# tencent-ailab/V-Express

Measured on AMD Instinct MI355X. Metric: decoded frames/sec at 512x512, 25 DDIM steps, higher is better.
Workload: dtype bf16; 1 GPU; 512x512, 16 frames (1 window(s) of 16, overlap 4), 25 DDIM steps, CFG 3.5, random-init UNet3D + ReferenceNet banks + sd-vae-ft-mse decode; frames=16, windows=1, parallelism=window x CFG-half units over 1 GPU(s)

## Files before the change

### v-express_amd/csrc/vx_norm.hip

```cpp
#include "vx_common.h"
#include "vx_gemm_common.h"
#include "../../include/vexpress_hip.h"

namespace {

constexpr int GN_THREADS = 256;
constexpr int GN_MAX_SETS = 2;

constexpr int GN_UNROLL = 4;
constexpr int GN_SUBS = 8;

struct GnPlan {
  const bf16_t* base[GN_MAX_SETS];
  int pstride[GN_MAX_SETS];
  int chunk[GN_MAX_SETS];
  int pl, pl_count;
};

__device__ __forceinline__ GnPlan gn_plan(const bf16_t* x1, int c1, const bf16_t* x2, int c2, int hw, int frame) {
  GnPlan P;
  const int nchunks = (c1 + c2) >> 3;
  const int tid = threadIdx.x;
  const int tp = nchunks < GN_THREADS ? nchunks : GN_THREADS;
  P.pl_count = GN_THREADS / tp;
  const int cc = tid % tp;
  P.pl = tid / tp;
  const bool active = P.pl < P.pl_count;
#pragma unroll
  for (int u = 0; u < GN_MAX_SETS; ++u) {
    const int chunk = cc + u * GN_THREADS;
    P.chunk[u] = chunk;
    const int ch = chunk * 8;
    if (active && chunk < nchunks) {
      if (ch < c1) {
        P.base[u] = x1 + (size_t)frame * hw * c1 + ch;
        P.pstride[u] = c1;
      } else {
        P.base[u] = x2 + (size_t)frame * hw * c2 + (ch - c1);
        P.pstride[u] = c2;
      }
    } else {
      P.base[u] = nullptr;
      P.pstride[u] = 0;
    }
  }
  return P;
}

__global__ __launch_bounds__(GN_THREADS) void gn_stats_kernel(const bf16_t* __restrict__ x1, int c1,
                                                              const bf16_t* __restrict__ x2, int c2, int hw,
                                                              int groups, int slices, int slice_pix,
                                                              float* __restrict__ ws) {
  extern __shared__ __attribute__((aligned(16))) char smem[];
  const int C = c1 + c2;
  const int bid = VX_XCD_ROWS ? xcd_remap(blockIdx.x, gridDim.x) : (int)blockIdx.x;
  const int frame = bid / slices, slice = bid % slices;
  const int tid = threadIdx.x;
  const GnPlan P = gn_plan(x1, c1, x2, c2, hw, frame);
  const int p_begin = slice * slice_pix;
  const int p_end = min(hw, p_begin + slice_pix);

  float s[GN_MAX_SETS][8], q[GN_MAX_SETS][8];
#pragma unroll
  for (int u = 0; u < GN_MAX_SETS; ++u)
#pragma unroll
    for (int e = 0; e < 8; ++e) s[u][e] = q[u][e] = 0.f;

#pragma unroll
  for (int u = 0; u < GN_MAX_SETS; ++u) {
    if (P.base[u] == nullptr) continue;
    const bf16_t* src = P.base[u];
    const int ps = P.pstride[u];
    int px = p_begin + P.pl;
    for (; px + (GN_UNROLL - 1) * P.pl_count < p_end; px += GN_UNROLL * P.pl_count) {
      uint4 raw[GN_UNROLL];
#pragma unroll
      for (int k = 0; k < GN_UNROLL; ++k)
        raw[k] = *reinterpret_cast<const uint4*>(src + (size_t)(px + k * P.pl_count) * ps);
#pragma unroll
      for (int k = 0; k < GN_UNROLL; ++k) {
        float f[8];
        unpack_bf16x8(raw[k], f);
#pragma unroll
        for (int e = 0; e < 8; ++e) {
          s[u][e] += f[e];
          q[u][e] += f[e] * f[e];
        }
      }
    }
    for (; px < p_end; px += P.pl_count) {
      float f[8];
      unpack_bf16x8(*reinterpret_cast<const uint4*>(src + (size_t)px * ps), f);
#pragma unroll
      for (int e = 0; e < 8; ++e) {
        s[u][e] += f[e];
        q[u][e] += f[e] * f[e];
      }
    }
  }
  float* part = reinterpret_cast<float*>(smem);
#pragma unroll
  for (int u = 0; u < GN_MAX_SETS; ++u) {
    if (P.base[u] == nullptr) continue;
#pragma unroll
    for (int e = 0; e < 8; ++e) {
      part[((size_t)P.pl * C + P.chunk[u] * 8 + e) * 2 + 0] = s[u][e];
      part[((size_t)P.pl * C + P.chunk[u] * 8 + e) * 2 + 1] = q[u][e];
    }
  }
  __syncthreads();
  for (int ch = tid; ch < C; ch += GN_THREADS) {
    float a = 0.f, b = 0.f;
    for (int l = 0; l < P.pl_count; ++l) {
      a += part[((size_t)l * C + ch) * 2 + 0];
      b += part[((size_t)l * C + ch) * 2 + 1];
    }
    part[(size_t)ch * 2 + 0] = a;
    part[(size_t)ch * 2 + 1] = b;
  }
  __syncthreads();
  const int cg = C / groups;
  for (int g = tid; g < groups; g += GN_THREADS) {
    float a = 0.f, b = 0.f;
    for (int j = 0; j < cg; ++j) {
      a += part[(size_t)(g * cg + j) * 2 + 0];
      b += part[(size_t)(g * cg + j) * 2 + 1];
    }
    float* o = ws + (((size_t)frame * slices + slice) * groups + g) * 2;
    o[0] = a;
    o[1] = b;
  }
}

__device__ __forceinline__ void gn_group_stats(const float* __restrict__ ws, int frame, int slices, int groups, int cg,
                                               int hw, float eps, float* gstat, double* dpart) {
  const int tid = threadIdx.x;
  for (int idx = tid; idx < groups * GN_SUBS; idx += GN_THREADS) {
    const int g = idx % groups, sub = idx / groups;
    double a = 0.0, b = 0.0;
    for (int sl = sub; sl < slices; sl += GN_SUBS) {
      const float2 o = *reinterpret_cast<const float2*>(ws + (((size_t)frame * slices + sl) * groups + g) * 2);
      a += (double)o.x;
      b += (double)o.y;
    }
    dpart[(sub * groups + g) * 2 + 0] = a;
    dpart[(sub * groups + g) * 2 + 1] = b;
  }
  __syncthreads();
  for (int g = tid; g < groups; g += GN_THREADS) {
    double a = 0.0, b = 0.0;
    for (int sub = 0; sub < GN_SUBS; ++sub) {
      a += dpart[(sub * groups + g) * 2 + 0];
      b += dpart[(sub * groups + g) * 2 + 1];
    }
    double cnt = (double)cg * (double)hw;
    double mean = a / cnt;
    double var = b / cnt - mean * mean;
    if (var < 0.0) var = 0.0;
    gstat[g * 2 + 0] = (float)mean;
    gstat[g * 2 + 1] = (float)(1.0 / sqrt(var + (double)eps));
  }
  __syncthreads();
}

constexpr int GN_FOLD_ROWS = GN_THREADS / 8;
__global__ __launch_bounds__(GN_THREADS) void gn_fold_linear_kernel(const float* __restrict__ ws, int hw, int slices,
                                                                    int groups, float eps,
                                                                    const float* __restrict__ gamma, int C,
                                                                    const bf16_t* __restrict__ w,
                                                                    const float* __restrict__ bias_beta, int n,
                                                                    bf16_t* __restrict__ w_out,
                                                                    float* __restrict__ bias_out) {
  extern __shared__ __attribute__((aligned(16))) char smem[];
  const int frame = blockIdx.y, tid = threadIdx.x;
  float* scale = reinterpret_cast<float*>(smem);
  float* meanc = scale + C;
  float* gstat = meanc + C;
  double* dpart = reinterpret_cast<double*>(gstat + 2 * groups);
  const int cg = C / groups;
  gn_group_stats(ws, frame, slices, groups, cg, hw, eps, gstat, dpart);
  for (int ch = tid; ch < C; ch += GN_THREADS) {
    const int g = ch / cg;
    scale[ch] = gamma[ch] * gstat[g * 2 + 1];
    meanc[ch] = gstat[g * 2 + 0];
  }
  __syncthreads();
  const int row = blockIdx.x * GN_FOLD_ROWS + (tid >> 3), sub = tid & 7;
  float dot = 0.f;
  if (row < n) {
    const bf16_t* src = w + (size_t)row * C;
    bf16_t* dst = w_out + ((size_t)frame * n + row) * C;
    for (int ch = sub * 8; ch < C; ch += 64) {
      float f[8];
      unpack_bf16x8(*reinterpret_cast<const uint4*>(src + ch), f);
#pragma unroll
      for (int e = 0; e < 8; ++e) f[e] *= scale[ch + e];
      const uint4 pk = pack_bf16x8(f);
      *reinterpret_cast<uint4*>(dst + ch) = pk;
      unpack_bf16x8(pk, f);
#pragma unroll
      for (int e = 0; e < 8; ++e) dot = fmaf(f[e], meanc[ch + e], dot);
    }
  }
  dot = wave_xor_sum(dot, 1);
  dot = wave_xor_sum(dot, 2);
  dot = wave_xor_sum(dot, 4);
  if (row < n && sub == 0) bias_out[(size_t)frame * n + row] = bias_beta[row] - dot;
}

__global__ __launch_bounds__(GN_THREADS) void gn_apply_kernel(const bf16_t* __restrict__ x1, int c1,
                                                              const bf16_t* __restrict__ x2, int c2, int hw,
                                                              int groups, float eps, const float* __restrict__ gamma,
                                                              const float* __restrict__ beta, int silu,
                                                              bf16_t* __restrict__ out, int slices, int slice_pix,
                                                              const float* __restrict__ ws, int width, int w_shift,
                                                              int out_pad, int stat_slices) {
  extern __shared__ __attribute__((aligned(16))) char smem[];
  const int C = c1 + c2;
  const int bid = VX_XCD_ROWS ? xcd_remap(blockIdx.x, gridDim.x) : (int)blockIdx.x;
  const int frame = bid / slices, slice = bid % slices;
  const int tid = threadIdx.x;
  float* scale = reinterpret_cast<float*>(smem);
  float* shift = scale + C;
  float* gstat = shift + C;
  double* dpart = reinterpret_cast<double*>(gstat + 2 * groups);
  const int cg = C / groups;
  gn_group_stats(ws, frame, stat_slices, groups, cg, hw, eps, gstat, dpart);
  for (int ch = tid; ch < C; ch += GN_THREADS) {
    int g = ch / cg;
    float sc = gamma[ch] * gstat[g * 2 + 1];
    scale[ch] = sc;
    shift[ch] = beta[ch] - gstat[g * 2 + 0] * sc;
  }
  __syncthreads();
  const GnPlan P = gn_plan(x1, c1, x2, c2, hw, frame);
  const int p_begin = slice * slice_pix;
  const int p_end = min(hw, p_begin + slice_pix);
  const int wp = width + 2 * out_pad;
  const int hp = hw / width + 2 * out_pad;
  bf16_t* const oframe = out + (size_t)frame * hp * wp * C;
  auto opix = [&](int px) {
    if (out_pad == 0) return px;
    const int y = w_shift >= 0 ? px >> w_shift : px / width;
    return (y + out_pad) * wp + (px - y * width) + out_pad;
  };
#pragma unroll
  for (int u = 0; u < GN_MAX_SETS; ++u) {
    if (P.base[u] == nullptr) continue;
    const bf16_t* src = P.base[u];
    const int ps = P.pstride[u];
    const int ch = P.chunk[u] * 8;
    float sc[8], sh[8];
#pragma unroll
    for (int e = 0; e < 8; ++e) {
      sc[e] = scale[ch + e];
      sh[e] = shift[ch + e];
    }
    auto emit = [&](const uint4& raw, int px) {
      float f[8];
      unpack_bf16x8(raw, f);
#pragma unroll
      for (int e = 0; e < 8; ++e) f[e] = f[e] * sc[e] + sh[e];
      if (silu == 1) {
#pragma unroll
        for (int e = 0; e < 8; ++e) f[e] = silu_f(f[e]);
      } else if (silu == 2) {
#pragma unroll
        for (int e = 0; e < 8; ++e) f[e] = gelu_f(f[e]);
      }
      *reinterpret_cast<uint4*>(oframe + (size_t)opix(px) * C + ch) = pack_bf16x8(f);
    };
    int px = p_begin + P.pl;
    for (; px + (GN_UNROLL - 1) * P.pl_count < p_end; px += GN_UNROLL * P.pl_count) {
      uint4 raw[GN_UNROLL];
#pragma unroll
      for (int k = 0; k < GN_UNROLL; ++k)
        raw[k] = *reinterpret_cast<const uint4*>(src + (size_t)(px + k * P.pl_count) * ps);
#pragma unroll
      for (int k = 0; k < GN_UNROLL; ++k) emit(raw[k], px + k * P.pl_count);
    }
    for (; px < p_end; px += P.pl_count) emit(*reinterpret_cast<const uint4*>(src + (size_t)px * ps), px);
  }
}

constexpr int LN_R = 4;

template <int MAXC>
__global__ __launch_bounds__(256) void layernorm_kernel(const bf16_t* __restrict__ x, int ldx, int rows, int c,
                                                        float eps, const float* __restrict__ gamma,
                                                        const float* __restrict__ beta,
                                                        const float* __restrict__ add, int add_rows_per_entry,
                                                        int add_entries, bf16_t* __restrict__ out, int ldo) {
  const int lane = threadIdx.x & 63;
  const int wave = blockIdx.x * 4 + (threadIdx.x >> 6);
  const int nwaves = gridDim.x * 4;
  const int nchunks = c >> 3;
  const float inv_c = 1.0f / (float)c;
  bool live[MAXC];
  float g[MAXC][8], b[MAXC][8];
#pragma unroll
  for (int u = 0; u < MAXC; ++u) {
    const int chunk = lane + u * 64;
    live[u] = chunk < nchunks;
    const int cs = live[u] ? chunk : 0;
    const float4 g0 = *reinterpret_cast<const float4*>(gamma + cs * 8);
    const float4 g1 = *reinterpret_cast<const float4*>(gamma + cs * 8 + 4);
    const float4 b0 = *reinterpret_cast<const float4*>(beta + cs * 8);
    const float4 b1 = *reinterpret_cast<const float4*>(beta + cs * 8 + 4);
    g[u][0] = g0.x; g[u][1] = g0.y; g[u][2] = g0.z; g[u][3] = g0.w;
    g[u][4] = g1.x; g[u][5] = g1.y; g[u][6] = g1.z; g[u][7] = g1.w;
    b[u][0] = b0.x; b[u][1] = b0.y; b[u][2] = b0.z; b[u][3] = b0.w;
    b[u][4] = b1.x; b[u][5] = b1.y; b[u][6] = b1.z; b[u][7] = b1.w;
  }
  for (int row0 = wave * LN_R; row0 < rows; row0 += nwaves * LN_R) {
    uint4 raw[LN_R][MAXC];
#pragma unroll
    for (int r = 0; r < LN_R; ++r) {
      const int row = min(row0 + r, rows - 1);
#pragma unroll
      for (int u = 0; u < MAXC; ++u) {
        const int chunk = live[u] ? lane + u * 64 : 0;
        raw[r][u] = *reinterpret_cast<const uint4*>(x + (size_t)row * ldx + chunk * 8);
      }
    }
    float sum[LN_R];
#pragma unroll
    for (int r = 0; r < LN_R; ++r) {
      sum[r] = 0.f;
#pragma unroll
      for (int u = 0; u < MAXC; ++u) {
        float v[8];
        unpack_bf16x8(raw[r][u], v);
        float t = ((v[0] + v[1]) + (v[2] + v[3])) + ((v[4] + v[5]) + (v[6] + v[7]));
        sum[r] += live[u] ? t : 0.f;
      }
    }
#pragma unroll
    for (int m = 32; m >= 1; m >>= 1)
#pragma unroll
      for (int r = 0; r < LN_R; ++r) sum[r] = wave_xor_sum(sum[r], m);
    float sq[LN_R];
#pragma unroll
    for (int r = 0; r < LN_R; ++r) {
      const float mean = sum[r] * inv_c;
      sq[r] = 0.f;
#pragma unroll
      for (int u = 0; u < MAXC; ++u) {
        float v[8];
        unpack_bf16x8(raw[r][u], v);
        float t = 0.f;
#pragma unroll
        for (int e = 0; e < 8; ++e) {
          const float d = v[e] - mean;
          t += d * d;
        }
        sq[r] += live[u] ? t : 0.f;
      }
    }
#pragma unroll
    for (int m = 32; m >= 1; m >>= 1)
#pragma unroll
      for (int r = 0; r < LN_R; ++r) sq[r] = wave_xor_sum(sq[r], m);
#pragma unroll
    for (int r = 0; r < LN_R; ++r) {
      const int row = row0 + r;
      if (row >= rows) break;
      const float mean = sum[r] * inv_c;
      const float rstd = rsqrtf(sq[r] * inv_c + eps);
      const float* addrow = nullptr;
      if (add != nullptr) addrow = add + (size_t)((row / add_rows_per_entry) % add_entries) * c;
#pragma unroll
      for (int u = 0; u < MAXC; ++u) {
        if (!live[u]) continue;
        const int chunk = lane + u * 64;
        float v[8], o[8];
        unpack_bf16x8(raw[r][u], v);
#pragma unroll
        for (int e = 0; e < 8; ++e) o[e] = (v[e] - mean) * rstd * g[u][e] + b[u][e];
        if (addrow != nullptr) {
          const float4 a0 = *reinterpret_cast<const float4*>(addrow + chunk * 8);
          const float4 a1 = *reinterpret_cast<const float4*>(addrow + chunk * 8 + 4);
          o[0] += a0.x; o[1] += a0.y; o[2] += a0.z; o[3] += a0.w;
          o[4] += a1.x; o[5] += a1.y; o[6] += a1.z; o[7] += a1.w;
        }
        *reinterpret_cast<uint4*>(out + (size_t)row * ldo + chunk * 8) = pack_bf16x8(o);
      }
    }
  }
}

template <int MAXC>
__global__ __launch_bounds__(256) void row_stats_kernel(const bf16_t* __restrict__ x, int ldx, int rows, int c, float eps,
                                                        float2* __restrict__ stats) {
  const int lane = threadIdx.x & 63;
  const int wave = blockIdx.x * 4 + (threadIdx.x >> 6);
  const int nwaves = gridDim.x * 4;
  const int nchunks = c >> 3;
  const float inv_c = 1.0f / (float)c;
  for (int row0 = wave * LN_R; row0 < rows; row0 += nwaves * LN_R) {
    uint4 raw[LN_R][MAXC];
#pragma unroll
    for (int r = 0; r < LN_R; ++r) {
      const int row = min(row0 + r, rows - 1);
#pragma unroll
      for (int u = 0; u < MAXC; ++u) {
        const int chunk = lane + u * 64 < nchunks ? lane + u * 64 : 0;
        raw[r][u] = *reinterpret_cast<const uint4*>(x + (size_t)row * ldx + chunk * 8);
      }
    }
    float sum[LN_R];
#pragma unroll
    for (int r = 0; r < LN_R; ++r) {
      sum[r] = 0.f;
#pragma unroll
      for (int u = 0; u < MAXC; ++u) {
        float v[8];
        unpack_bf16x8(raw[r][u], v);
        const float t = ((v[0] + v[1]) + (v[2] + v[3])) + ((v[4] + v[5]) + (v[6] + v[7]));
        sum[r] += lane + u * 64 < nchunks ? t : 0.f;
      }
    }
#pragma unroll
    for (int m = 32; m >= 1; m >>= 1)
#pragma unroll
      for (int r = 0; r < LN_R; ++r) sum[r] = wave_xor_sum(sum[r], m);
    float sq[LN_R];
#pragma unroll
    for (int r = 0; r < LN_R; ++r) {
      const float mean = sum[r] * inv_c;
      sq[r] = 0.f;
#pragma unroll
      for (int u = 0; u < MAXC; ++u) {
        float v[8];
        unpack_bf16x8(raw[r][u], v);
        float t = 0.f;
#pragma unroll
        for (int e = 0; e < 8; ++e) {
          const float d = v[e] - mean;
          t += d * d;
        }
        sq[r] += lane + u * 64 < nchunks ? t : 0.f;
      }
    }
#pragma unroll
    for (int m = 32; m >= 1; m >>= 1)
#pragma unroll
      for (int r = 0; r < LN_R; ++r) sq[r] = wave_xor_sum(sq[r], m);
    if (lane < LN_R && row0 + lane < rows) {
      float mean = 0.f, var = 0.f;
#pragma unroll
      for (int r = 0; r < LN_R; ++r)
        if (lane == r) {
          mean = sum[r] * inv_c;
          var = sq[r] * inv_c;
        }
      stats[row0 + lane] = make_float2(mean, rsqrtf(var + eps));
    }
  }
}

template <int MAXC, bool NORM>
__global__ __launch_bounds__(256) void layernorm_fp8_kernel(const bf16_t* __restrict__ x, int ldx, int rows, int c,
                                                            float eps, const float* __restrict__ gamma,
                                                            const float* __restrict__ beta,
                                                            const float* __restrict__ add, int add_rows_per_entry,
                                                            int add_entries, uint8_t* __restrict__ out8, int ldo8,
                                                            float* __restrict__ scale) {
  const int lane = threadIdx.x & 63;
  const int wave = blockIdx.x * 4 + (threadIdx.x >> 6);
  const int nwaves = gridDim.x * 4;
  const int nchunks = c >> 3, ochunks = ldo8 >> 3;
  const float inv_c = 1.0f / (float)c;
  for (int row = wave; row < rows; row += nwaves) {
    float y[MAXC][8];
    float sum = 0.f;
#pragma unroll
    for (int u = 0; u < MAXC; ++u) {
      const int chunk = lane + u * 64;
      if (chunk < nchunks) {
        unpack_bf16x8(*reinterpret_cast<const uint4*>(x + (size_t)row * ldx + chunk * 8), y[u]);
      } else {
#pragma unroll
        for (int e = 0; e < 8; ++e) y[u][e] = 0.f;
      }
      sum += ((y[u][0] + y[u][1]) + (y[u][2] + y[u][3])) + ((y[u][4] + y[u][5]) + (y[u][6] + y[u][7]));
    }
    if (NORM) {
#pragma unroll
      for (int m = 32; m >= 1; m >>= 1) sum = wave_xor_sum(sum, m);
      const float mean = sum * inv_c;
      float sq = 0.f;
#pragma unroll
      for (int u = 0; u < MAXC; ++u) {
        if (lane + u * 64 < nchunks) {
#pragma unroll
          for (int e = 0; e < 8; ++e) {
            const float d = y[u][e] - mean;
            sq += d * d;
          }
        }
      }
#pragma unroll
      for (int m = 32; m >= 1; m >>= 1) sq = wave_xor_sum(sq, m);
      const float rstd = rsqrtf(sq * inv_c + eps);
      const float* addrow = add != nullptr ? add + (size_t)((row / add_rows_per_entry) % add_entries) * c : nullptr;
#pragma unroll
      for (int u = 0; u < MAXC; ++u) {
        const int chunk = lane + u * 64;
        if (chunk < nchunks) {
#pragma unroll
          for (int e = 0; e < 8; ++e) {
            float o = (y[u][e] - mean) * rstd * gamma[chunk * 8 + e] + beta[chunk * 8 + e];
            if (addrow != nullptr) o += addrow[chunk * 8 + e];
            y[u][e] = o;
          }
        }
      }
    }
    float amax = 0.f;
#pragma unroll
    for (int u = 0; u < MAXC; ++u)
#pragma unroll
      for (int e = 0; e < 8; ++e) amax = fmaxf(amax, fabsf(y[u][e]));
#pragma unroll
    for (int m = 32; m >= 1; m >>= 1) amax = wave_xor_max(amax, m);
    const float sc = amax > 0.f ? amax * (1.0f / 448.0f) : 1.0f;
    const float inv = 1.0f / sc;
    if (lane == 0) scale[row] = sc;
#pragma unroll
    for (int u = 0; u < MAXC; ++u) {
      const int chunk = lane + u * 64;
      if (chunk < ochunks) {
        int w0 = 0, w1 = 0;
        w0 = __builtin_amdgcn_cvt_pk_fp8_f32(y[u][0] * inv, y[u][1] * inv, w0, false);
        w0 = __builtin_amdgcn_cvt_pk_fp8_f32(y[u][2] * inv, y[u][3] * inv, w0, true);
        w1 = __builtin_amdgcn_cvt_pk_fp8_f32(y[u][4] * inv, y[u][5] * inv, w1, false);
        w1 = __builtin_amdgcn_cvt_pk_fp8_f32(y[u][6] * inv, y[u][7] * inv, w1, true);
        *reinterpret_cast<uint2*>(out8 + (size_t)row * ldo8 + chunk * 8) = make_uint2((uint32_t)w0, (uint32_t)w1);
      }
    }
  }
}

}

extern "C" int64_t vx_groupnorm_ws_floats(int frames, int slices, int groups) {
  return (int64_t)frames * slices * groups * 2;
}

extern "C" int vx_groupnorm(const void* x1, int c1, const void* x2, int c2, int frames, int hw, int groups, float eps,
                            const float* gamma, const float* beta, int silu, void* out, float* ws, int slices,
                            int width, int out_pad, void* stream_) {
  hipStream_t stream = (hipStream_t)stream_;
  const int C = c1 + c2;
  VX_REQUIRE(x1 != nullptr && out != nullptr && ws != nullptr && gamma != nullptr && beta != nullptr,
             "vx_groupnorm: null pointer");
  VX_REQUIRE((c2 == 0) == (x2 == nullptr), "vx_groupnorm: x2/c2 mismatch");
  VX_REQUIRE(c1 > 0 && (c1 % 8) == 0 && (c2 % 8) == 0, "vx_groupnorm: channels must be multiples of 8");
  VX_REQUIRE(groups > 0 && (C % groups) == 0, "vx_groupnorm: C=%d not divisible by groups=%d", C, groups);
  VX_REQUIRE(C <= 8 * GN_THREADS * GN_MAX_SETS, "vx_groupnorm: C=%d too large", C);
  VX_REQUIRE(frames > 0 && hw > 0 && slices > 0 && slices <= hw, "vx_groupnorm: bad geometry");
  VX_REQUIRE(silu >= 0 && silu <= 2, "vx_groupnorm: activation code %d (0 none, 1 SiLU, 2 erf-GELU)", silu);
  VX_REQUIRE(out_pad >= 0 && (out_pad == 0 || (width > 0 && hw % width == 0)),
             "vx_groupnorm: padded output needs the image width (hw=%d width=%d)", hw, width);
  if (out_pad == 0) width = hw;
  int w_shift = -1;
  for (int sft = 0; sft < 31; ++sft)
    if ((1 << sft) == width) w_shift = sft;
  const int slice_pix = ceil_div(hw, slices);
  const int nchunks = C / 8;
  const int tp = nchunks < GN_THREADS ? nchunks : GN_THREADS;
  const int pl_count = GN_THREADS / tp;
  size_t smem_stats = (size_t)pl_count * C * 2 * sizeof(float);
  size_t smem_apply = (size_t)(2 * C + 2 * groups) * sizeof(float) + (size_t)GN_SUBS * groups * 2 * sizeof(double);
  VX_REQUIRE(smem_stats <= 64 * 1024, "vx_groupnorm: stats LDS %zu too large", smem_stats);
  hipLaunchKernelGGL(gn_stats_kernel, dim3(frames * slices), dim3(GN_THREADS), smem_stats, stream,
                     (const bf16_t*)x1, c1, (const bf16_t*)x2, c2, hw, groups, slices, slice_pix, ws);
  int rc = vx_check_launch("vx_groupnorm(stats)");
  if (rc) return rc;
  static int amax = -1;
  if (amax < 0) {
    const char* e = getenv("VX_GN_APPLY_SLICES");
    amax = e ? atoi(e) : 64;
    if (amax < 1) amax = 1;
  }
  const int aslices = slices < amax ? slices : amax;
  const int apix = ceil_div(hw, aslices);
  hipLaunchKernelGGL(gn_apply_kernel, dim3(frames * aslices), dim3(GN_THREADS), smem_apply, stream,
                     (const bf16_t*)x1, c1, (const bf16_t*)x2, c2, hw, groups, eps, gamma, beta, silu,
                     (bf16_t*)out, aslices, apix, (const float*)ws, width, w_shift, out_pad, slices);
  return vx_check_launch("vx_groupnorm(apply)");
}

extern "C" int vx_groupnorm_apply(const void* x1, int c1, const void* x2, int c2, int frames, int hw, int groups,
                                  float eps, const float* gamma, const float* beta, int silu, void* out,
                                  const float* ws, int stat_slices, int slices, int width, int out_pad, void* stream_) {
  hipStream_t stream = (hipStream_t)stream_;
  const int C = c1 + c2;
  VX_REQUIRE(x1 != nullptr && out != nullptr && ws != nullptr && gamma != nullptr && beta != nullptr,
             "vx_groupnorm_apply: null pointer");
  VX_REQUIRE((c2 == 0) == (x2 == nullptr), "vx_groupnorm_apply: x2/c2 mismatch");
  VX_REQUIRE(c1 > 0 && (c1 % 8) == 0 && (c2 % 8) == 0, "vx_groupnorm_apply: channels must be multiples of 8");
  VX_REQUIRE(groups > 0 && (C % groups) == 0, "vx_groupnorm_apply: C=%d not divisible by groups=%d", C, groups);
  VX_REQUIRE(C <= 8 * GN_THREADS * GN_MAX_SETS, "vx_groupnorm_apply: C=%d too large", C);
  VX_REQUIRE(frames > 0 && hw > 0 && slices > 0 && slices <= hw && stat_slices > 0, "vx_groupnorm_apply: bad geometry");
  VX_REQUIRE(silu >= 0 && silu <= 2, "vx_groupnorm_apply: activation code %d (0 none, 1 SiLU, 2 erf-GELU)", silu);
  VX_REQUIRE(out_pad >= 0 && (out_pad == 0 || (width > 0 && hw % width == 0)),
             "vx_groupnorm_apply: padded output needs the image width (hw=%d width=%d)", hw, width);
  if (out_pad == 0) width = hw;
  int w_shift = -1;
  for (int sft = 0; sft < 31; ++sft)
    if ((1 << sft) == width) w_shift = sft;
  const size_t smem_apply = (size_t)(2 * C + 2 * groups) * sizeof(float) + (size_t)GN_SUBS * groups * 2 * sizeof(double);
  const int apix = ceil_div(hw, slices);
  hipLaunchKernelGGL(gn_apply_kernel, dim3(frames * slices), dim3(GN_THREADS), smem_apply, stream, (const bf16_t*)x1, c1,
                     (const bf16_t*)x2, c2, hw, groups, eps, gamma, beta, silu, (bf16_t*)out, slices, apix, ws, width,
                     w_shift, out_pad, stat_slices);
  return vx_check_launch("vx_groupnorm_apply");
}

extern "C" int vx_groupnorm_stats(const void* x1, int c1, const void* x2, int c2, int frames, int hw, int groups,
                                  float* ws, int slices, void* stream_) {
  hipStream_t stream = (hipStream_t)stream_;
  const int C = c1 + c2;
  VX_REQUIRE(x1 != nullptr && ws != nullptr, "vx_groupnorm_stats: null pointer");
  VX_REQUIRE((c2 == 0) == (x2 == nullptr), "vx_groupnorm_stats: x2/c2 mismatch");
  VX_REQUIRE(c1 > 0 && (c1 % 8) == 0 && (c2 % 8) == 0, "vx_groupnorm_stats: channels must be multiples of 8");
  VX_REQUIRE(groups > 0 && (C % groups) == 0, "vx_groupnorm_stats: C=%d not divisible by groups=%d", C, groups);
  VX_REQUIRE(C <= 8 * GN_THREADS * GN_MAX_SETS, "vx_groupnorm_stats: C=%d too large", C);
  VX_REQUIRE(frames > 0 && hw > 0 && slices > 0 && slices <= hw, "vx_groupnorm_stats: bad geometry");
  const int slice_pix = ceil_div(hw, slices);
  const int nchunks = C / 8;
  const int tp = nchunks < GN_THREADS ? nchunks : GN_THREADS;
  const size_t smem_stats = (size_t)(GN_THREADS / tp) * C * 2 * sizeof(float);
  VX_REQUIRE(smem_stats <= 64 * 1024, "vx_groupnorm_stats: stats LDS %zu too large", smem_stats);
  hipLaunchKernelGGL(gn_stats_kernel, dim3(frames * slices), dim3(GN_THREADS), smem_stats, stream,
                     (const bf16_t*)x1, c1, (const bf16_t*)x2, c2, hw, groups, slices, slice_pix, ws);
  return vx_check_launch("vx_groupnorm_stats");
}

extern "C" int vx_groupnorm_fold_linear(const float* ws, int frames, int hw, int slices, int groups, float eps,
                                        const float* gamma, int c, const void* w, const float* bias_beta, int n,
                                        void* w_out, float* bias_out, void* stream_) {
  hipStream_t stream = (hipStream_t)stream_;
  VX_REQUIRE(ws != nullptr && gamma != nullptr && w != nullptr && bias_beta != nullptr && w_out != nullptr &&
                 bias_out != nullptr, "vx_groupnorm_fold_linear: null pointer");
  VX_REQUIRE(frames > 0 && hw > 0 && slices > 0 && n > 0 && c > 0 && (c % 8) == 0 && groups > 0 && (c % groups) == 0,
             "vx_groupnorm_fold_linear: bad geometry (c=%d groups=%d n=%d)", c, groups, n);
  const size_t smem = (size_t)(2 * c + 2 * groups) * sizeof(float) + (size_t)GN_SUBS * groups * 2 * sizeof(double);
  VX_REQUIRE(smem <= 64 * 1024, "vx_groupnorm_fold_linear: c=%d too large", c);
  hipLaunchKernelGGL(gn_fold_linear_kernel, dim3(ceil_div(n, GN_FOLD_ROWS), frames), dim3(GN_THREADS), smem, stream, ws,
                     hw, slices, groups, eps, gamma, c, (const bf16_t*)w, bias_beta, n, (bf16_t*)w_out, bias_out);
  return vx_check_launch("vx_groupnorm_fold_linear");
}

extern "C" int vx_layernorm(const void* x, int ldx, int rows, int c, float eps, const float* gamma,
                            const float* beta, const float* add, int add_rows_per_entry, int add_entries, void* out,
                            int ldo, void* stream_) {
  hipStream_t stream = (hipStream_t)stream_;
  VX_REQUIRE(x != nullptr && out != nullptr && gamma != nullptr && beta != nullptr, "vx_layernorm: null pointer");
  VX_REQUIRE(rows > 0 && c > 0 && (c % 8) == 0 && (ldx % 8) == 0 && (ldo % 8) == 0, "vx_layernorm: bad shape");
  VX_REQUIRE(add == nullptr || (add_rows_per_entry > 0 && add_entries > 0), "vx_layernorm: bad add table");
  const int nchunks = c / 8;
  int nblk = ceil_div(rows, 4 * LN_R);
  if (nblk > 4096) nblk = 4096;
  dim3 grid(nblk), block(256);
#define VX_LN(MAXC)                                                                                              \
  hipLaunchKernelGGL(layernorm_kernel<MAXC>, grid, block, 0, stream, (const bf16_t*)x, ldx, rows, c, eps, gamma, \
                     beta, add, add_rows_per_entry, add_entries, (bf16_t*)out, ldo)
  if (nchunks <= 64) VX_LN(1);
  else if (nchunks <= 128) VX_LN(2);
  else if (nchunks <= 192) VX_LN(3);
  else if (nchunks <= 256) VX_LN(4);
  else {
    vx_set_error("vx_layernorm: c=%d exceeds 2048", c);
    return VX_ERR_UNSUPPORTED;
  }
#undef VX_LN
  return vx_check_launch("vx_layernorm");
}

extern "C" int vx_layernorm_fp8(const void* x, int ldx, int rows, int c, float eps, const float* gamma,
                                const float* beta, const float* add, int add_rows_per_entry, int add_entries,
                                void* out8, int ldo8, float* scale, void* stream_) {
  hipStream_t stream = (hipStream_t)stream_;
  VX_REQUIRE(x != nullptr && out8 != nullptr && scale != nullptr, "vx_layernorm_fp8: null pointer");
  VX_REQUIRE((gamma == nullptr) == (beta == nullptr), "vx_layernorm_fp8: gamma and beta come together");
  VX_REQUIRE(rows > 0 && c > 0 && (c % 8) == 0 && (ldx % 8) == 0 && (ldo8 % 16) == 0 && ldo8 >= c,
             "vx_layernorm_fp8: bad shape (c=%d ldx=%d ldo8=%d)", c, ldx, ldo8);
  VX_REQUIRE(add == nullptr || (gamma != nullptr && add_rows_per_entry > 0 && add_entries > 0),
             "vx_layernorm_fp8: bad add table");
  const int ochunks = ldo8 / 8;
  int nblk = ceil_div(rows, 4);
  if (nblk > 8192) nblk = 8192;
  dim3 grid(nblk), block(256);
#define VX_LN8(MAXC)                                                                                                  \
  do {                                                                                                                \
    if (gamma != nullptr)                                                                                             \
      hipLaunchKernelGGL((layernorm_fp8_kernel<MAXC, true>), grid, block, 0, stream, (const bf16_t*)x, ldx, rows, c,  \
                         eps, gamma, beta, add, add_rows_per_entry, add_entries, (uint8_t*)out8, ldo8, scale);        \
    else                                                                                                              \
      hipLaunchKernelGGL((layernorm_fp8_kernel<MAXC, false>), grid, block, 0, stream, (const bf16_t*)x, ldx, rows, c, \
                         eps, gamma, beta, add, add_rows_per_entry, add_entries, (uint8_t*)out8, ldo8, scale);        \
  } while (0)
  if (ochunks <= 64) VX_LN8(1);
  else if (ochunks <= 128) VX_LN8(2);
  else if (ochunks <= 192) VX_LN8(3);
  else if (ochunks <= 256) VX_LN8(4);
  else {
    vx_set_error("vx_layernorm_fp8: c=%d exceeds 2048", c);
    return VX_ERR_UNSUPPORTED;
  }
#undef VX_LN8
  return vx_check_launch("vx_layernorm_fp8");
}

__global__ __launch_bounds__(256) void row_stats_parts_kernel(const bf16_t* __restrict__ x, int ldx, int rows, int c,
                                                              float4* __restrict__ stats) {
  const int lane = threadIdx.x & 63, half = lane >> 5, l32 = lane & 31;
  const int hc = c >> 1;
  for (int row = blockIdx.x * 4 + (threadIdx.x >> 6); row < rows; row += gridDim.x * 4) {
    const bf16_t* src = x + (size_t)row * ldx + half * hc;
    float sm = 0.f, sq = 0.f;
    for (int ch = l32 * 8; ch < hc; ch += 32 * 8) {
      float v[8];
      unpack_bf16x8(*reinterpret_cast<const uint4*>(src + ch), v);
      sm += ((v[0] + v[1]) + (v[2] + v[3])) + ((v[4] + v[5]) + (v[6] + v[7]));
#pragma unroll
      for (int e = 0; e < 8; ++e) sq = fmaf(v[e], v[e], sq);
    }
#pragma unroll
    for (int m = 16; m >= 1; m >>= 1) {
      sm = wave_xor_sum(sm, m);
      sq = wave_xor_sum(sq, m);
    }
    const float s1 = __shfl(sm, 32, 64), q1 = __shfl(sq, 32, 64);
    if (lane == 0) stats[row] = make_float4(sm, sq, s1, q1);
  }
}

extern "C" int vx_row_stats_parts(const void* x, int ldx, int rows, int c, float* stats, void* stream_) {
  VX_REQUIRE(x != nullptr && stats != nullptr, "vx_row_stats_parts: null pointer");
  VX_REQUIRE(rows > 0 && c > 0 && (c % 16) == 0 && (ldx % 8) == 0, "vx_row_stats_parts: bad shape");
  int nblk = ceil_div(rows, 4);
  if (nblk > 8192) nblk = 8192;
  hipLaunchKernelGGL(row_stats_parts_kernel, dim3(nblk), dim3(256), 0, (hipStream_t)stream_, (const bf16_t*)x, ldx, rows, c,
                     reinterpret_cast<float4*>(stats));
  return vx_check_launch("vx_row_stats_parts");
}

__global__ __launch_bounds__(256) void row_stats_finalize_kernel(const float4* __restrict__ parts, int rows, float inv_c,
                                                                 float eps, float2* __restrict__ stats) {
  for (int r = blockIdx.x * 256 + threadIdx.x; r < rows; r += gridDim.x * 256) {
    const float4 t = parts[r];
    const float mean = (t.x + t.z) * inv_c;
    float var = (t.y + t.w) * inv_c - mean * mean;
    var = var > 0.f ? var : 0.f;
    stats[r] = make_float2(mean, 1.0f / sqrtf(var + eps));
  }
}

extern "C" int vx_row_stats_finalize(const float* parts, int rows, int c, float eps, float* stats, void* stream_) {
  VX_REQUIRE(parts != nullptr && stats != nullptr && rows > 0 && c > 0 && eps > 0.f, "vx_row_stats_finalize: bad arguments");
  int nblk = ceil_div(rows, 256);
  if (nblk > 2048) nblk = 2048;
  hipLaunchKernelGGL(row_stats_finalize_kernel, dim3(nblk), dim3(256), 0, (hipStream_t)stream_,
                     reinterpret_cast<const float4*>(parts), rows, 1.0f / (float)c, eps, reinterpret_cast<float2*>(stats));
  return vx_check_launch("vx_row_stats_finalize");
}

extern "C" int vx_row_stats(const void* x, int ldx, int rows, int c, float eps, float* stats, void* stream_) {
  hipStream_t stream = (hipStream_t)stream_;
  VX_REQUIRE(x != nullptr && stats != nullptr, "vx_row_stats: null pointer");
  VX_REQUIRE(rows > 0 && c > 0 && (c % 8) == 0 && (ldx % 8) == 0, "vx_row_stats: bad shape");
  const int nchunks = c / 8;
  int nblk = ceil_div(rows, 4 * LN_R);
  if (nblk > 4096) nblk = 4096;
  dim3 grid(nblk), block(256);
#define VX_RS(MAXC)                                                                                        \
  hipLaunchKernelGGL(row_stats_kernel<MAXC>, grid, block, 0, stream, (const bf16_t*)x, ldx, rows, c, eps, \
                     reinterpret_cast<float2*>(stats))
  if (nchunks <= 64) VX_RS(1);
  else if (nchunks <= 128) VX_RS(2);
  else if (nchunks <= 192) VX_RS(3);
  else if (nchunks <= 256) VX_RS(4);
  else {
    vx_set_error("vx_row_stats: c=%d exceeds 2048", c);
    return VX_ERR_UNSUPPORTED;
  }
#undef VX_RS
  return vx_check_launch("vx_row_stats");
}
```

Baseline: 14.43 frames/s.

## Add one-pass fused GroupNorm and small-spatial apply kernels

```diff
diff --git a/v-express_amd/csrc/vx_norm.hip b/v-express_amd/csrc/vx_norm.hip
--- a/v-express_amd/csrc/vx_norm.hip
+++ b/v-express_amd/csrc/vx_norm.hip
@@ -132,9 +132,44 @@
   }
 }
 
+__device__ __forceinline__ void gn_finish_stats(double a, double b, int cg, int hw, float eps, float* gs) {
+  double cnt = (double)cg * (double)hw;
+  double mean = a / cnt;
+  double var = b / cnt - mean * mean;
+  if (var < 0.0) var = 0.0;
+  gs[0] = (float)mean;
+  gs[1] = (float)(1.0 / sqrt(var + (double)eps));
+}
+
+__device__ __forceinline__ void gn_scale_shift(float gamma, float beta, const float* gs, float* scale, float* shift) {
+  float sc = gamma * gs[1];
+  *scale = sc;
+  *shift = beta - gs[0] * sc;
+}
+
 __device__ __forceinline__ void gn_group_stats(const float* __restrict__ ws, int frame, int slices, int groups, int cg,
                                                int hw, float eps, float* gstat, double* dpart) {
   const int tid = threadIdx.x;
+  if (slices <= GN_SUBS) {
+    for (int g = tid; g < groups; g += GN_THREADS) {
+      float2 o[GN_SUBS];
+#pragma unroll
+      for (int sl = 0; sl < GN_SUBS; ++sl)
+        o[sl] = sl < slices ? *reinterpret_cast<const float2*>(ws + (((size_t)frame * slices + sl) * groups + g) * 2)
+                            : make_float2(0.f, 0.f);
+      double a = 0.0, b = 0.0;
+#pragma unroll
+      for (int sl = 0; sl < GN_SUBS; ++sl) {
+        if (sl < slices) {
+          a += (double)o[sl].x;
+          b += (double)o[sl].y;
+        }
+      }
+      gn_finish_stats(a, b, cg, hw, eps, gstat + g * 2);
+    }
+    __syncthreads();
+    return;
+  }
   for (int idx = tid; idx < groups * GN_SUBS; idx += GN_THREADS) {
     const int g = idx % groups, sub = idx / groups;
     double a = 0.0, b = 0.0;
@@ -153,14 +188,24 @@
       a += dpart[(sub * groups + g) * 2 + 0];
       b += dpart[(sub * groups + g) * 2 + 1];
     }
-    double cnt = (double)cg * (double)hw;
-    double mean = a / cnt;
-    double var = b / cnt - mean * mean;
-    if (var < 0.0) var = 0.0;
-    gstat[g * 2 + 0] = (float)mean;
-    gstat[g * 2 + 1] = (float)(1.0 / sqrt(var + (double)eps));
+    gn_finish_stats(a, b, cg, hw, eps, gstat + g * 2);
   }
   __syncthreads();
+}
+
+__device__ __forceinline__ uint4 gn_emit(const uint4& raw, const float* sc, const float* sh, int silu) {
+  float f[8];
+  unpack_bf16x8(raw, f);
+#pragma unroll
+  for (int e = 0; e < 8; ++e) f[e] = f[e] * sc[e] + sh[e];
+  if (silu == 1) {
+#pragma unroll
+    for (int e = 0; e < 8; ++e) f[e] = silu_f(f[e]);
+  } else if (silu == 2) {
+#pragma unroll
+    for (int e = 0; e < 8; ++e) f[e] = gelu_f(f[e]);
+  }
+  return pack_bf16x8(f);
 }
 
 constexpr int GN_FOLD_ROWS = GN_THREADS / 8;
@@ -226,12 +271,7 @@
   double* dpart = reinterpret_cast<double*>(gstat + 2 * groups);
   const int cg = C / groups;
   gn_group_stats(ws, frame, stat_slices, groups, cg, hw, eps, gstat, dpart);
-  for (int ch = tid; ch < C; ch += GN_THREADS) {
-    int g = ch / cg;
-    float sc = gamma[ch] * gstat[g * 2 + 1];
-    scale[ch] = sc;
-    shift[ch] = beta[ch] - gstat[g * 2 + 0] * sc;
-  }
+  for (int ch = tid; ch < C; ch += GN_THREADS) gn_scale_shift(gamma[ch], beta[ch], gstat + (ch / cg) * 2, scale + ch, shift + ch);
   __syncthreads();
   const GnPlan P = gn_plan(x1, c1, x2, c2, hw, frame);
   const int p_begin = slice * slice_pix;
@@ -257,18 +297,7 @@
       sh[e] = shift[ch + e];
     }
     auto emit = [&](const uint4& raw, int px) {
-      float f[8];
-      unpack_bf16x8(raw, f);
-#pragma unroll
-      for (int e = 0; e < 8; ++e) f[e] = f[e] * sc[e] + sh[e];
-      if (silu == 1) {
-#pragma unroll
-        for (int e = 0; e < 8; ++e) f[e] = silu_f(f[e]);
-      } else if (silu == 2) {
-#pragma unroll
-        for (int e = 0; e < 8; ++e) f[e] = gelu_f(f[e]);
-      }
-      *reinterpret_cast<uint4*>(oframe + (size_t)opix(px) * C + ch) = pack_bf16x8(f);
+      *reinterpret_cast<uint4*>(oframe + (size_t)opix(px) * C + ch) = gn_emit(raw, sc, sh, silu);
     };
     int px = p_begin + P.pl;
     for (; px + (GN_UNROLL - 1) * P.pl_count < p_end; px += GN_UNROLL * P.pl_count) {
@@ -280,6 +309,214 @@
       for (int k = 0; k < GN_UNROLL; ++k) emit(raw[k], px + k * P.pl_count);
     }
     for (; px < p_end; px += P.pl_count) emit(*reinterpret_cast<const uint4*>(src + (size_t)px * ps), px);
+  }
+}
+
+constexpr int GNF_PIX = 8;
+constexpr int GNF_MAX_PIX = 16;
+constexpr int GNF_THREADS = 512;
+constexpr int GNF_MIN_THREADS = 128;
+
+__global__ __launch_bounds__(GNF_THREADS) void gn_fused_kernel(const bf16_t* __restrict__ x1, int c1,
+                                                               const bf16_t* __restrict__ x2, int c2, int hw, int groups,
+                                                               float eps, const float* __restrict__ gamma,
+                                                               const float* __restrict__ beta, int silu,
+                                                               bf16_t* __restrict__ out, int slices, int slice_pix,
+                                                               float* __restrict__ ws, int width, int w_shift, int out_pad,
+                                                               int gpb, int bchunks, int nseg) {
+  extern __shared__ __attribute__((aligned(16))) char smem[];
+  const int C = c1 + c2, cg = C / groups;
+  const int nsplit = groups / gpb;
+  const int bid = VX_XCD_ROWS ? xcd_remap(blockIdx.x, gridDim.x) : (int)blockIdx.x;
+  const int frame = bid / nsplit, split = bid % nsplit;
+  const int tid = threadIdx.x, nthr = blockDim.x;
+  const int bC = bchunks * 8;
+  float* part = reinterpret_cast<float*>(smem);
+  float* gpart = part + (size_t)slices * bC * 2;
+  float* gstat = gpart + slices * gpb * 2;
+  const int cl = tid % bchunks, series = tid / bchunks;
+  const int seg = series % nseg, sl = series / nseg;
+  const int ch = (split * bchunks + cl) * 8;
+  const int p_begin = sl * slice_pix + seg * GNF_PIX;
+  int npix = 0;
+  if (sl < slices) npix = min(min(hw, (sl + 1) * slice_pix) - p_begin, GNF_PIX);
+  if (npix < 0) npix = 0;
+  const bf16_t* src;
+  int ps;
+  if (ch < c1) {
+    src = x1 + ((size_t)frame * hw + p_begin) * c1 + ch;
+    ps = c1;
+  } else {
+    src = x2 + ((size_t)frame * hw + p_begin) * c2 + (ch - c1);
+    ps = c2;
+  }
+  uint4 raw[GNF_PIX];
+#pragma unroll
+  for (int k = 0; k < GNF_PIX; ++k)
+    if (k < npix) raw[k] = *reinterpret_cast<const uint4*>(src + (size_t)k * ps);
+  float gm[8], bt[8];
+#pragma unroll
+  for (int e = 0; e < 8; ++e) {
+    gm[e] = gamma[ch + e];
+    bt[e] = beta[ch + e];
+  }
+  for (int r = 0; r < nseg; ++r) {
+    if (seg == r && sl < slices) {
+      float4* acc = reinterpret_cast<float4*>(part + ((size_t)sl * bC + cl * 8) * 2);
+      float s[8], q[8];
+      if (r == 0) {
+#pragma unroll
+        for (int e = 0; e < 8; ++e) s[e] = q[e] = 0.f;
+      } else {
+        const float4 a0 = acc[0], a1 = acc[1], a2 = acc[2], a3 = acc[3];
+        s[0] = a0.x; q[0] = a0.y; s[1] = a0.z; q[1] = a0.w; s[2] = a1.x; q[2] = a1.y; s[3] = a1.z; q[3] = a1.w;
+        s[4] = a2.x; q[4] = a2.y; s[5] = a2.z; q[5] = a2.w; s[6] = a3.x; q[6] = a3.y; s[7] = a3.z; q[7] = a3.w;
+      }
+#pragma unroll
+      for (int k = 0; k < GNF_PIX; ++k) {
+        if (k < npix) {
+          float f[8];
+          unpack_bf16x8(raw[k], f);
+#pragma unroll
+          for (int e = 0; e < 8; ++e) {
+            s[e] += f[e];
+            q[e] += f[e] * f[e];
+          }
+        }
+      }
+      acc[0] = make_float4(s[0], q[0], s[1], q[1]);
+      acc[1] = make_float4(s[2], q[2], s[3], q[3]);
+      acc[2] = make_float4(s[4], q[4], s[5], q[5]);
+      acc[3] = make_float4(s[6], q[6], s[7], q[7]);
+    }
+    __syncthreads();
+  }
+  for (int idx = tid; idx < slices * gpb; idx += nthr) {
+    const int gl = idx % gpb, s2 = idx / gpb;
+    const float2* p = reinterpret_cast<const float2*>(part + ((size_t)s2 * bC + gl * cg) * 2);
+    float a = 0.f, b = 0.f;
+    int j = 0;
+    for (; j + 8 <= cg; j += 8) {
+      float2 v[8];
+#pragma unroll
+      for (int k = 0; k < 8; ++k) v[k] = p[j + k];
+#pragma unroll
+      for (int k = 0; k < 8; ++k) {
+        a += v[k].x;
+        b += v[k].y;
+      }
+    }
+    for (; j < cg; ++j) {
+      a += p[j].x;
+      b += p[j].y;
+    }
+    gpart[idx * 2 + 0] = a;
+    gpart[idx * 2 + 1] = b;
+    float* o = ws + (((size_t)frame * slices + s2) * groups + split * gpb + gl) * 2;
+    o[0] = a;
+    o[1] = b;
+  }
+  __syncthreads();
+  for (int gl = tid; gl < gpb; gl += nthr) {
+    double a = 0.0, b = 0.0;
+    for (int s2 = 0; s2 < slices; ++s2) {
+      a += (double)gpart[(s2 * gpb + gl) * 2 + 0];
+      b += (double)gpart[(s2 * gpb + gl) * 2 + 1];
+    }
+    gn_finish_stats(a, b, cg, hw, eps, gstat + gl * 2);
+  }
+  __syncthreads();
+  if (npix == 0) return;
+  float sc[8], sh[8];
+#pragma unroll
+  for (int e = 0; e < 8; ++e) gn_scale_shift(gm[e], bt[e], gstat + ((cl * 8 + e) / cg) * 2, sc + e, sh + e);
+  const int wp = width + 2 * out_pad;
+  const int hp = hw / width + 2 * out_pad;
+  bf16_t* const oframe = out + (size_t)frame * hp * wp * C + ch;
+#pragma unroll
+  for (int k = 0; k < GNF_PIX; ++k) {
+    if (k < npix) {
+      const int px = p_begin + k;
+      int op = px;
+      if (out_pad != 0) {
+        const int y = w_shift >= 0 ? px >> w_shift : px / width;
+        op = (y + out_pad) * wp + (px - y * width) + out_pad;
+      }
+      *reinterpret_cast<uint4*>(oframe + (size_t)op * C) = gn_emit(raw[k], sc, sh, silu);
+    }
+  }
+}
+
+constexpr int GNA_PIX = 4;
+constexpr int GNA_ITEMS = GNA_PIX * GN_MAX_SETS;
+constexpr int GNA_CH = 8 * GN_MAX_SETS;
+
+__global__ __launch_bounds__(GN_THREADS) void gn_apply_small_kernel(const bf16_t* __restrict__ x1, int c1,
+                                                                    const bf16_t* __restrict__ x2, int c2, int hw,
+                                                                    int groups, float eps, const float* __restrict__ gamma,
+                                                                    const float* __restrict__ beta, int silu,
+                                                                    bf16_t* __restrict__ out, int pieces,
+                                                                    const float* __restrict__ ws, int width, int w_shift,
+                                                                    int out_pad, int stat_slices) {
+  extern __shared__ __attribute__((aligned(16))) char smem[];
+  const int C = c1 + c2, nchunks = C >> 3;
+  const int bid = VX_XCD_ROWS ? xcd_remap(blockIdx.x, gridDim.x) : (int)blockIdx.x;
+  const int frame = bid / pieces, piece = bid % pieces;
+  const int tid = threadIdx.x;
+  float* scale = reinterpret_cast<float*>(smem);
+  float* shift = scale + C;
+  float* gstat = shift + C;
+  double* dpart = reinterpret_cast<double*>(gstat + 2 * groups);
+  const int cg = C / groups;
+  const int p_begin = piece * GNA_PIX;
+  const int nitems = min(GNA_PIX, hw - p_begin) * nchunks;
+  uint4 raw[GNA_ITEMS];
+#pragma unroll
+  for (int k = 0; k < GNA_ITEMS; ++k) {
+    const int i = tid + k * GN_THREADS;
+    if (i < nitems) {
+      const int p = i / nchunks, ch = (i - p * nchunks) * 8;
+      const size_t pix = (size_t)frame * hw + p_begin + p;
+      raw[k] = *reinterpret_cast<const uint4*>(ch < c1 ? x1 + pix * c1 + ch : x2 + pix * c2 + (ch - c1));
+    }
+  }
+  float gm[GNA_CH], bt[GNA_CH];
+#pragma unroll
+  for (int j = 0; j < GNA_CH; ++j) {
+    const int c = tid + j * GN_THREADS;
+    if (c < C) {
+      gm[j] = gamma[c];
+      bt[j] = beta[c];
+    }
+  }
+  gn_group_stats(ws, frame, stat_slices, groups, cg, hw, eps, gstat, dpart);
+#pragma unroll
+  for (int j = 0; j < GNA_CH; ++j) {
+    const int c = tid + j * GN_THREADS;
+    if (c < C) gn_scale_shift(gm[j], bt[j], gstat + (c / cg) * 2, scale + c, shift + c);
+  }
+  __syncthreads();
+  const int wp = width + 2 * out_pad;
+  const int hp = hw / width + 2 * out_pad;
+  bf16_t* const oframe = out + (size_t)frame * hp * wp * C;
+#pragma unroll
+  for (int k = 0; k < GNA_ITEMS; ++k) {
+    const int i = tid + k * GN_THREADS;
+    if (i < nitems) {
+      const int p = i / nchunks, ch = (i - p * nchunks) * 8;
+      const int px = p_begin + p;
+      int op = px;
+      if (out_pad != 0) {
+        const int y = w_shift >= 0 ? px >> w_shift : px / width;
+        op = (y + out_pad) * wp + (px - y * width) + out_pad;
+      }
+      float sc[8], sh[8];
+      const float4 s0 = *reinterpret_cast<const float4*>(scale + ch), s1 = *reinterpret_cast<const float4*>(scale + ch + 4);
+      const float4 h0 = *reinterpret_cast<const float4*>(shift + ch), h1 = *reinterpret_cast<const float4*>(shift + ch + 4);
+      sc[0] = s0.x; sc[1] = s0.y; sc[2] = s0.z; sc[3] = s0.w; sc[4] = s1.x; sc[5] = s1.y; sc[6] = s1.z; sc[7] = s1.w;
+      sh[0] = h0.x; sh[1] = h0.y; sh[2] = h0.z; sh[3] = h0.w; sh[4] = h1.x; sh[5] = h1.y; sh[6] = h1.z; sh[7] = h1.w;
+      *reinterpret_cast<uint4*>(oframe + (size_t)op * C + ch) = gn_emit(raw[k], sc, sh, silu);
+    }
   }
 }
 
@@ -542,6 +779,48 @@
   }
 }
 
+}
+
+static int gn_small_mask() {
+  static int mask = -1;
+  if (mask < 0) {
+    const char* e = getenv("VX_GN_SMALL");
+    mask = e ? (atoi(e) & 3) : 3;
+  }
+  return mask;
+}
+
+static bool gn_fused_plan(int C, int hw, int slices, int slice_pix, int groups, int* gpb, int* bchunks, int* nseg, int* threads,
+                          size_t* smem) {
+  if (!(gn_small_mask() & 1)) return false;
+  const int nchunks = C / 8, cg = C / groups;
+  if (nchunks <= GN_THREADS / 2 || slice_pix > GNF_MAX_PIX || slices > GN_SUBS) return false;
+  const int ns = ceil_div(slice_pix, GNF_PIX);
+  for (int g = 1; g <= groups; ++g) {
+    if (groups % g != 0 || (g * cg) % 8 != 0) continue;
+    const int bc = g * cg / 8, t = bc * slices * ns;
+    if (t < GNF_MIN_THREADS && g < groups) continue;
+    const size_t sm = ((size_t)slices * bc * 8 * 2 + (size_t)slices * g * 2 + (size_t)g * 2) * sizeof(float);
+    if (t > GNF_THREADS || sm > 64 * 1024) return false;
+    *gpb = g;
+    *bchunks = bc;
+    *nseg = ns;
+    *threads = (t + 63) / 64 * 64;
+    *smem = sm;
+    return true;
+  }
+  return false;
+}
+
+static bool gn_apply_small_ok(int C, int hw) { return (gn_small_mask() & 2) && hw <= 64; }
+
+static void gn_launch_apply_small(const void* x1, int c1, const void* x2, int c2, int frames, int hw, int groups, float eps,
+                                  const float* gamma, const float* beta, int silu, void* out, const float* ws, int stat_slices,
+                                  int width, int w_shift, int out_pad, size_t smem, hipStream_t stream) {
+  const int pieces = ceil_div(hw, GNA_PIX);
+  hipLaunchKernelGGL(gn_apply_small_kernel, dim3(frames * pieces), dim3(GN_THREADS), smem, stream, (const bf16_t*)x1, c1,
+                     (const bf16_t*)x2, c2, hw, groups, eps, gamma, beta, silu, (bf16_t*)out, pieces, ws, width, w_shift, out_pad,
+                     stat_slices);
 }
 
 extern "C" int64_t vx_groupnorm_ws_floats(int frames, int slices, int groups) {
@@ -574,10 +853,23 @@
   size_t smem_stats = (size_t)pl_count * C * 2 * sizeof(float);
   size_t smem_apply = (size_t)(2 * C + 2 * groups) * sizeof(float) + (size_t)GN_SUBS * groups * 2 * sizeof(double);
   VX_REQUIRE(smem_stats <= 64 * 1024, "vx_groupnorm: stats LDS %zu too large", smem_stats);
+  int gpb, bchunks, nseg, fthreads;
+  size_t smem_fused;
+  if (gn_fused_plan(C, hw, slices, slice_pix, groups, &gpb, &bchunks, &nseg, &fthreads, &smem_fused)) {
+    hipLaunchKernelGGL(gn_fused_kernel, dim3(frames * (groups / gpb)), dim3(fthreads), smem_fused, stream, (const bf16_t*)x1, c1,
+                       (const bf16_t*)x2, c2, hw, groups, eps, gamma, beta, silu, (bf16_t*)out, slices, slice_pix, ws, width,
+                       w_shift, out_pad, gpb, bchunks, nseg);
+    return vx_check_launch("vx_groupnorm(one pass)");
+  }
   hipLaunchKernelGGL(gn_stats_kernel, dim3(frames * slices), dim3(GN_THREADS), smem_stats, stream,
                      (const bf16_t*)x1, c1, (const bf16_t*)x2, c2, hw, groups, slices, slice_pix, ws);
   int rc = vx_check_launch("vx_groupnorm(stats)");
   if (rc) return rc;
+  if (gn_apply_small_ok(C, hw)) {
+    gn_launch_apply_small(x1, c1, x2, c2, frames, hw, groups, eps, gamma, beta, silu, out, ws, slices, width, w_shift, out_pad,
+                          smem_apply, stream);
+    return vx_check_launch("vx_groupnorm(apply)");
+  }
   static int amax = -1;
   if (amax < 0) {
     const char* e = getenv("VX_GN_APPLY_SLICES");
@@ -612,6 +904,11 @@
   for (int sft = 0; sft < 31; ++sft)
     if ((1 << sft) == width) w_shift = sft;
   const size_t smem_apply = (size_t)(2 * C + 2 * groups) * sizeof(float) + (size_t)GN_SUBS * groups * 2 * sizeof(double);
+  if (gn_apply_small_ok(C, hw)) {
+    gn_launch_apply_small(x1, c1, x2, c2, frames, hw, groups, eps, gamma, beta, silu, out, ws, stat_slices, width, w_shift,
+                          out_pad, smem_apply, stream);
+    return vx_check_launch("vx_groupnorm_apply");
+  }
   const int apix = ceil_div(hw, slices);
   hipLaunchKernelGGL(gn_apply_kernel, dim3(frames * slices), dim3(GN_THREADS), smem_apply, stream, (const bf16_t*)x1, c1,
                      (const bf16_t*)x2, c2, hw, groups, eps, gamma, beta, silu, (bf16_t*)out, slices, apix, ws, width,
```

New measurement: 14.47 frames/s, median of 6. No clear change (+0.3%).
